# aiortc/aioquic

Hardware: AMD Instinct MI355X
Metric: GiB/s device-resident AEAD protect+unprotect, 1200B packets, 1/2/4/8 MI355X (higher is better)
Workload: dtype u8

## Files before the change

### aioquic_amd/csrc/qpp_device.h

```cpp
#pragma once

#include <hip/hip_runtime.h>
#include <stdint.h>

#include "../../include/quic_pp.h"
#include "qpp_gh5.h"
#include "qpp_te4.h"

namespace qpp {


extern __constant__ AesTables c_aes;


struct KeySlot {
    uint32_t suite;
    uint32_t key_phase;
    uint32_t nr;
    uint32_t rsv;
    uint32_t iv[4];
    uint32_t rk[60];
    uint32_t hrk[60];
    uint32_t rkr[60];
    uint32_t pad[4];
};
static_assert(sizeof(KeySlot) == 768, "KeySlot layout");

constexpr int kGhashPowers = 4;
constexpr int kGhashPowBytes = 32 * 16 * 16;

constexpr int kGh5Off = kGhashPowers * kGhashPowBytes;
constexpr int kGhPowCount = 192;
constexpr int kGhPowBytes = kGhPowCount * 16;
constexpr int kGhashTabBytes = kGh5Off + kGh5Bytes;
__device__ __host__ __forceinline__ size_t gh_powers_off(uint32_t cap, uint32_t slot)
{
    return (size_t)cap * kGhashTabBytes + (size_t)slot * kGhPowBytes;
}
// ... 180 lines not shown
        return (*(const uint32_t *)(te + addr<0>(s)) >> 8) & 0xffu;
    }
    __device__ __forceinline__ uint32_t f1(uint32_t s) const
    {
        return *(const uint32_t *)(te + addr<1>(s)) & 0xff00u;
    }
    __device__ __forceinline__ uint32_t f2(uint32_t s) const
    {
        return *(const uint32_t *)(te + 128 + addr<2>(s)) & 0xff0000u;
    }
    __device__ __forceinline__ uint32_t f3(uint32_t s) const
    {
        return *(const uint32_t *)(te + 128 + addr<3>(s)) & 0xff000000u;
    }
    __device__ __forceinline__ uint32_t fr0(uint32_t s) const { return *(const uint32_t *)(te + addr<0>(s)); }
    __device__ __forceinline__ uint32_t fr1(uint32_t s) const { return *(const uint32_t *)(te + addr<1>(s)); }
    __device__ __forceinline__ uint32_t fr2(uint32_t s) const { return *(const uint32_t *)(te + 128 + addr<2>(s)); }
    __device__ __forceinline__ uint32_t fr3(uint32_t s) const { return *(const uint32_t *)(te + 128 + addr<3>(s)); }
};

struct LdsTe4 {
    static constexpr bool kFourTables = true;
    const uint8_t *te;
    uint32_t lo;
    template <int R, bool HI>
    __device__ __forceinline__ uint32_t addr(uint32_t s) const
    {
        return __builtin_amdgcn_perm(s, lo, (HI ? 0x0c020000u : 0x0c0c0000u) | ((4u + R) << 8));
    }
    __device__ __forceinline__ uint32_t t0(uint32_t s) const { return *(const uint32_t *)(te + addr<0, false>(s)); }
    __device__ __forceinline__ uint32_t t1(uint32_t s) const { return *(const uint32_t *)(te + 128 + addr<1, false>(s)); }
    __device__ __forceinline__ uint32_t t2(uint32_t s) const { return *(const uint32_t *)(te + addr<2, true>(s)); }
    __device__ __forceinline__ uint32_t t3(uint32_t s) const { return *(const uint32_t *)(te + 128 + addr<3, true>(s)); }
    __device__ __forceinline__ uint32_t f0(uint32_t s) const { return (fr0(s) >> 8) & 0xffu; }
    __device__ __forceinline__ uint32_t f1(uint32_t s) const { return fr1(s) & 0xff00u; }
    __device__ __forceinline__ uint32_t f2(uint32_t s) const { return fr2(s) & 0xff0000u; }
    __device__ __forceinline__ uint32_t f3(uint32_t s) const { return fr3(s) & 0xff000000u; }
    __device__ __forceinline__ uint32_t fr0(uint32_t s) const { return *(const uint32_t *)(te + addr<0, false>(s)); }
    __device__ __forceinline__ uint32_t fr1(uint32_t s) const { return *(const uint32_t *)(te + addr<1, false>(s)); }
    __device__ __forceinline__ uint32_t fr2(uint32_t s) const { return *(const uint32_t *)(te + 128 + addr<2, false>(s)); }
    __device__ __forceinline__ uint32_t fr3(uint32_t s) const { return *(const uint32_t *)(te + 128 + addr<3, false>(s)); }
};

__device__ __forceinline__ uint32_t fin_col(uint32_t r0, uint32_t r1, uint32_t r2, uint32_t r3, uint32_t k)
{
    const uint32_t lo = __builtin_amdgcn_perm(r1, r0, 0x0c0c0501u);
    const uint32_t hi = __builtin_amdgcn_perm(r3, r2, 0x07020c0cu);
    return __builtin_amdgcn_bitop3_b32(lo, hi, k, 0x56);
}

struct ConstTe {
    __device__ __forceinline__ uint32_t t0(uint32_t s) const { return c_aes.te0[s & 255]; }
    __device__ __forceinline__ uint32_t t1(uint32_t s) const { return rotl(c_aes.te0[(s >> 8) & 255], 8); }
    __device__ __forceinline__ uint32_t t2(uint32_t s) const { return rotl(c_aes.te0[(s >> 16) & 255], 16); }
    __device__ __forceinline__ uint32_t t3(uint32_t s) const { return rotl(c_aes.te0[s >> 24], 24); }
    __device__ __forceinline__ uint32_t t2r(uint32_t s) const { return c_aes.te0[(s >> 16) & 255]; }
    __device__ __forceinline__ uint32_t t3r(uint32_t s) const { return rotl(c_aes.te0[s >> 24], 8); }
    __device__ __forceinline__ uint32_t f0(uint32_t s) const { return c_aes.sbox[s & 255]; }
    __device__ __forceinline__ uint32_t f1(uint32_t s) const { return (uint32_t)c_aes.sbox[(s >> 8) & 255] << 8; }
    __device__ __forceinline__ uint32_t f2(uint32_t s) const { return (uint32_t)c_aes.sbox[(s >> 16) & 255] << 16; }
    __device__ __forceinline__ uint32_t f3(uint32_t s) const { return (uint32_t)c_aes.sbox[s >> 24] << 24; }
};

template <int NR, int R0, bool KROT = false, class TE>
__device__ __forceinline__ u32x4 aes_rounds(u32x4 st, const uint32_t *rk, const TE &T)
{
// ... 60 lines not shown
    constexpr int kNext1 = 0x39, kNext2 = 0x4E, kNext3 = 0x93;
    uint32_t k[NR + 1];
#pragma unroll
    for (int r = 0; r <= NR; ++r) k[r] = rk[4 * r + sub];
    uint32_t s = (sub == 0 ? in.x : sub == 1 ? in.y : sub == 2 ? in.z : in.w) ^ k[0];
#pragma unroll
    for (int r = 1; r < NR; ++r) {
        const uint32_t s1 = quad_perm<kNext1>(s), s2 = quad_perm<kNext2>(s), s3 = quad_perm<kNext3>(s);
        s = xor3(xor3(T.t0(s), T.t1(s1), T.t2(s2)), T.t3(s3), k[r]);
    }
    const uint32_t s1 = quad_perm<kNext1>(s), s2 = quad_perm<kNext2>(s), s3 = quad_perm<kNext3>(s);
    s = (T.f0(s) | T.f1(s1) | T.f2(s2) | T.f3(s3)) ^ k[NR];
    return u32x4{quad_perm<0x00>(s), quad_perm<0x55>(s), quad_perm<0xAA>(s), quad_perm<0xFF>(s)};
}

struct CtrCache {
    uint32_t c0, d0, d1, d2, d3;
};

template <class TE>
__device__ __forceinline__ CtrCache ctr_cache(u32x4 nonce, const uint32_t *rk, const TE &T)
{
    const uint32_t s0 = nonce.x ^ rk[0], s1 = nonce.y ^ rk[1], s2 = nonce.z ^ rk[2], s3 = rk[3];
    const uint32_t c0 = xor3(T.t0(s0), T.t1(s1), T.t2(s2)) ^ rk[4];
    const uint32_t u1 = xor3(xor3(T.t0(s1), T.t1(s2), T.t2(s3)), T.t3(s0), rk[5]);
    const uint32_t u2 = xor3(xor3(T.t0(s2), T.t1(s3), T.t2(s0)), T.t3(s1), rk[6]);
    const uint32_t u3 = xor3(xor3(T.t0(s3), T.t1(s0), T.t2(s1)), T.t3(s2), rk[7]);
    return CtrCache{c0, xor3(T.t1(u1), T.t2(u2), T.t3(u3)) ^ rk[8],
                    xor3(T.t0(u1), T.t1(u2), T.t2(u3)) ^ rk[9],
                    xor3(T.t0(u2), T.t1(u3), T.t3(u1)) ^ rk[10],
                    xor3(T.t0(u3), T.t2(u1), T.t3(u2)) ^ rk[11]};
}

template <int NR, class TE>
__device__ __forceinline__ u32x4 aes_ctr(const CtrCache &c, uint32_t cb, const uint32_t *rk,
                                         const TE &T)
{
    const uint32_t u0 = c.c0 ^ T.t3(rk[3] ^ (cb << 24));
    const u32x4 v = {c.d0 ^ T.t0(u0), c.d1 ^ T.t3(u0), c.d2 ^ T.t2(u0), c.d3 ^ T.t1(u0)};
    return aes_rounds<NR, 3, true>(v, rk, T);
}

template <int NR, class TE>
__device__ __forceinline__ void aes_ctr2(const CtrCache &c, uint32_t cb0, uint32_t cb1,
                                         const uint32_t *rk, const TE &T, u32x4 &o0, u32x4 &o1)
{
    const uint32_t x0 = T.t3(rk[3] ^ (cb0 << 24)), x1 = T.t3(rk[3] ^ (cb1 << 24));
    __builtin_amdgcn_sched_barrier(0);
    const uint32_t u0 = c.c0 ^ x0, u1 = c.c0 ^ x1;
    const uint32_t v0 = T.t0(u0), v1 = T.t3(u0), v2 = T.t2(u0), v3 = T.t1(u0);
    const uint32_t w0 = T.t0(u1), w1 = T.t3(u1), w2 = T.t2(u1), w3 = T.t1(u1);
    __builtin_amdgcn_sched_barrier(0);
    uint32_t s[2][4] = {{c.d0 ^ v0, c.d1 ^ v1, c.d2 ^ v2, c.d3 ^ v3},
                        {c.d0 ^ w0, c.d1 ^ w1, c.d2 ^ w2, c.d3 ^ w3}};
#pragma unroll
    for (int r = 3; r < NR; ++r) {
        const uint32_t *k = rk + 4 * r;
        uint32_t e[2][16];
#pragma unroll
        for (int b = 0; b < 2; ++b) {
#pragma unroll
            for (int col = 0; col < 4; ++col) {
                e[b][4 * col + 0] = T.t0(s[b][col]);
                e[b][4 * col + 1] = T.t1(s[b][(col + 1) & 3]);
                if constexpr (TE::kFourTables) {
                    e[b][4 * col + 2] = T.t2(s[b][(col + 2) & 3]);
                    e[b][4 * col + 3] = T.t3(s[b][(col + 3) & 3]);
                } else {
                    e[b][4 * col + 2] = T.t2r(s[b][(col + 2) & 3]);
                    e[b][4 * col + 3] = T.t3r(s[b][(col + 3) & 3]);
                }
            }
        }
        __builtin_amdgcn_sched_barrier(0);
#pragma unroll
        for (int b = 0; b < 2; ++b) {
#pragma unroll
            for (int col = 0; col < 4; ++col) {
                if constexpr (TE::kFourTables)
                    s[b][col] = te_col4(e[b][4 * col], e[b][4 * col + 1], e[b][4 * col + 2], e[b][4 * col + 3], k[col]);
                else
                    s[b][col] = te_col2(e[b][4 * col], e[b][4 * col + 1], e[b][4 * col + 2], e[b][4 * col + 3], k[col]);
            }
        }
    }
    const uint32_t *k = rk + 4 * NR;
    uint32_t f[2][16];
#pragma unroll
    for (int b = 0; b < 2; ++b) {
#pragma unroll
        for (int col = 0; col < 4; ++col) {
            f[b][4 * col + 0] = T.fr0(s[b][col]);
            f[b][4 * col + 1] = T.fr1(s[b][(col + 1) & 3]);
            f[b][4 * col + 2] = T.fr2(s[b][(col + 2) & 3]);
            f[b][4 * col + 3] = T.fr3(s[b][(col + 3) & 3]);
        }
    }
    __builtin_amdgcn_sched_barrier(0);
    uint32_t o[2][4];
#pragma unroll
    for (int b = 0; b < 2; ++b) {
#pragma unroll
        for (int col = 0; col < 4; ++col)
            o[b][col] = fin_col(f[b][4 * col], f[b][4 * col + 1], f[b][4 * col + 2], f[b][4 * col + 3], k[col]);
    }
    o0 = u32x4{o[0][0], o[0][1], o[0][2], o[0][3]};
    o1 = u32x4{o[1][0], o[1][1], o[1][2], o[1][3]};
}


__device__ __forceinline__ u32x4 ghash_mul(u32x4 x, const uint8_t *lds, uint32_t tab)
{
    u32x4 acc = {0, 0, 0, 0};
    uint32_t xw[4] = {x.x, x.y, x.z, x.w};
#pragma unroll 1
    for (int d = 0; d < 4; ++d) {
        const uint32_t w = d == 0 ? xw[0] : d == 1 ? xw[1] : d == 2 ? xw[2] : xw[3];
        uint32_t hi = w & 0xF0F0F0F0u;
        uint32_t lo = (w << 4) & 0xF0F0F0F0u;
#pragma unroll
        for (int b = 0; b < 4; ++b) {
            const int wlo = 2 * (4 * d + b), whi = wlo + 1;
            const uint32_t sel = 0x0c0c0c00u | (uint32_t)b;
            uint32_t alo = __builtin_amdgcn_perm(0u, lo, sel);
            uint32_t ahi = __builtin_amdgcn_perm(0u, hi, sel);
            u32x4 e0 = *(const u32x4 *)(lds + tab + wlo * 256 + alo);
            u32x4 e1 = *(const u32x4 *)(lds + tab + whi * 256 + ahi);
            acc = xor3(acc, e0, e1);
        }
    }
    return acc;
}

template <int W0, int W1>
struct Gh5Grp {
    u32x2 lo[W1 - W0], hi[W1 - W0];
    __device__ __forceinline__ void issue(const uint32_t (&xw)[4], const uint8_t *base, uint32_t tsel)
    {
#pragma unroll
        for (int i = 0; i < W1 - W0; ++i) {
            const int w = W0 + i, sb = 5 * w, d = sb >> 5, off = sb & 31;
            uint32_t e;
            if (off <= 27) asm("v_bfe_u32 %0, %1, %2, 5" : "=v"(e) : "v"(xw[d]), "i"(off));
            else if (d < 3) e = __builtin_amdgcn_alignbit(xw[d + 1], xw[d], off) & 31u;
            else e = xw[3] >> off;
            const uint32_t a = (e << 3) | tsel;
            lo[i] = *(const u32x2 *)(base + w * 256 + a);
            hi[i] = *(const u32x2 *)(base + kGh5Hi + w * 256 + a);
        }
    }
    __device__ __forceinline__ void consume(u32x4 &acc) const
    {
        constexpr int n = W1 - W0;
#pragma unroll
        for (int i = 0; i + 1 < n; i += 2) {
            acc.x = xor3(acc.x, lo[i].x, lo[i + 1].x);
            acc.y = xor3(acc.y, lo[i].y, lo[i + 1].y);
            acc.z = xor3(acc.z, hi[i].x, hi[i + 1].x);
            acc.w = xor3(acc.w, hi[i].y, hi[i + 1].y);
        }
        if constexpr (n & 1) {
            acc.x ^= lo[n - 1].x;
            acc.y ^= lo[n - 1].y;
            acc.z ^= hi[n - 1].x;
            acc.w ^= hi[n - 1].y;
        }
    }
};

template <template <int, int> class Grp, class... In>
__device__ __forceinline__ u32x4 gh5_pipeline(const In &...in)
{
    u32x4 acc = {0, 0, 0, 0};
#define QPP_SB() __builtin_amdgcn_sched_barrier(0)
    {
        Grp<0, 5> a;
        Grp<5, 9> b;
        Grp<9, 14> c;
        Grp<14, 18> d;
        Grp<18, 22> e;
        Grp<22, kGh5Windows> f;
        a.issue(in...);
        b.issue(in...);
        QPP_SB();
        a.consume(acc);
        QPP_SB();
        c.issue(in...);
        QPP_SB();
        b.consume(acc);
        QPP_SB();
        d.issue(in...);
        QPP_SB();
        c.consume(acc);
        QPP_SB();
        e.issue(in...);
        QPP_SB();
        d.consume(acc);
        QPP_SB();
        f.issue(in...);
        QPP_SB();
        e.consume(acc);
        QPP_SB();
        f.consume(acc);
        QPP_SB();
    }
#undef QPP_SB
    return acc;
}
__device__ __forceinline__ u32x4 ghash_mul_lds5(u32x4 x, const uint8_t *base, uint32_t tsel)
{
    const uint32_t xw[4] = {x.x, x.y, x.z, x.w};
    return gh5_pipeline<Gh5Grp>(xw, base, tsel);
}

__device__ __forceinline__ u32x4 ghash_mul_h4(u32x4 x, const uint8_t *base, uint32_t tsel)
{
    return ghash_mul_lds5(x, base, tsel);
}

template <int W0, int W1>
struct Gh5GrpC : Gh5Grp<W0, W1> {
    template <int i = 0>
    __device__ __forceinline__ void issue(const Gh5In &in, const uint8_t *base)
    {
        if constexpr (i < W1 - W0) {
            constexpr int w = W0 + i;
            const uint32_t a = gh5_addr<w>(in);
            this->lo[i] = *(const u32x2 *)(base + w * 256 + a);
            this->hi[i] = *(const u32x2 *)(base + kGh5Hi + w * 256 + a);
            issue<i + 1>(in, base);
        }
    }
};
__device__ __forceinline__ u32x4 ghash_mul_lds5c(u32x4 x, const uint8_t *base)
{
    const Gh5In in(x.x, x.y, x.z, x.w);
    return gh5_pipeline<Gh5GrpC>(in, base);
}

__device__ __forceinline__ u32x4 ghash_mul_global(u32x4 x, const uint8_t *tab)
{
    u32x4 acc = {0, 0, 0, 0};
    uint32_t xw[4] = {x.x, x.y, x.z, x.w};
#pragma unroll 1
    for (int d = 0; d < 4; ++d) {
        const uint32_t w = d == 0 ? xw[0] : d == 1 ? xw[1] : d == 2 ? xw[2] : xw[3];
        uint32_t hi = w & 0xF0F0F0F0u;
        uint32_t lo = (w << 4) & 0xF0F0F0F0u;
#pragma unroll
        for (int b = 0; b < 4; ++b) {
            const int wlo = 2 * (4 * d + b), whi = wlo + 1;
            const uint32_t sel = 0x0c0c0c00u | (uint32_t)b;
            const uint32_t alo = __builtin_amdgcn_perm(0u, lo, sel);
            const uint32_t ahi = __builtin_amdgcn_perm(0u, hi, sel);
            u32x4 e0 = *(const u32x4 *)(tab + wlo * 256 + alo);
            u32x4 e1 = *(const u32x4 *)(tab + whi * 256 + ahi);
            acc = xor3(acc, e0, e1);
        }
    }
    return acc;
}

__device__ inline u32x4 gf128_mul_slow(u32x4 x, u32x4 y)
{
    uint64_t xh = (uint64_t)bswap(x.x) << 32 | bswap(x.y), xl = (uint64_t)bswap(x.z) << 32 | bswap(x.w);
    uint64_t vh = (uint64_t)bswap(y.x) << 32 | bswap(y.y), vl = (uint64_t)bswap(y.z) << 32 | bswap(y.w);
    uint64_t zh = 0, zl = 0;
    for (int i = 0; i < 128; ++i) {
        uint64_t bit = i < 64 ? (xh >> (63 - i)) & 1 : (xl >> (127 - i)) & 1;
        if (bit) { zh ^= vh; zl ^= vl; }
// ... 11 lines not shown
```

### aioquic_amd/csrc/qpp_engine.hip

```cpp
#include <hip/hip_runtime.h>

#include "qpp_chacha.h"
#include "qpp_gf128.h"
#include "qpp_device.h"
#include "qpp_hkdf.h"
#include "qpp_internal.h"
#include "qpp_phase.h"

namespace qpp {

__constant__ AesTables c_aes = kAesTables;

constexpr int kSetupWG = 256;
constexpr int kScratch = 112;
constexpr int kScrEj0 = 48, kScrPark = 64, kScrHdr = 96;
constexpr uint32_t kNoSlot = 0xffffffffu;
constexpr int kChachaWpe = 4;

constexpr int kChRegion = 64 * 16 + 16;
constexpr int kChStage = 4 * kChRegion;

constexpr int kPwOne = 0, kPw1 = 1, kPw8 = 6, kPw13 = 7, kPwEntries = 11;
constexpr int kChCarryAt = 7;

// ... 447 lines not shown
        }
        if (rb & 1) __builtin_amdgcn_raw_buffer_store_b8((unsigned char)t, r, o + (rb & 2), 0, 0);
    }
}

__device__ __forceinline__ void write_header_v(const Pkt &P, int sub, bool masked, int rlen, u32x4 h0,
                                               bool have_h0)
{
    const int n_a = (P.hlen + 15) >> 4;
    for (int q = sub; q < n_a; q += 4) {
        const int nb = min(16, P.hlen - 16 * q);
        u32x4 h = (q == 0 && have_h0) ? h0 : ld_win(P.src + 16 * q, nb, P.src, P.src + rlen);
        if (masked) h ^= hp_pattern(16 * q, P.mask, P.fbm, P.pn_off, P.pn_len);
        st_part(P.dst + 16 * q, h, nb);
    }
}

template <int NR, bool ENC, int BPL, int SUITE, bool PRIO, bool CLDS = false>
__device__ __forceinline__ u32x4 gcm_packet(const Pkt &P, const KeySlot *ks, const u32x4 h0,
                                            const uint32_t *rk, int sub, const GhashTabs &G,
                                            const uint8_t *te, const Bufs &B, uint32_t ioff, uint32_t ooff,
                                            u32x4 &got_tag)
{
    typedef std::conditional_t<CLDS, LdsTe4, LdsTe> Te;
    auto te_now = [&]() -> Te { return Te{te, (lane_fresh() & 31) * 4 | (CLDS ? 0x10000u : 0u)}; };
    const Te T = te_now();
    const int hlen = P.hlen, clen = P.clen;
    const int n_a = (hlen + 15) >> 4, n_c = (clen + 15) >> 4, za = n_a > 0 ? 1 : 0;
    const int n_g = za + n_c + 1, pad = gcm_pad<BPL>(n_g), S = (n_g + pad) / (4 * BPL);
    const int rlen = hlen + clen + (ENC ? 0 : QPP_TAG_LEN);
    const bool tiny = rlen < 16;
    const uint32_t t4 = CLDS ? 0u : G.t4();
    auto mul_h4 = [&](u32x4 x) -> u32x4 {
        if constexpr (CLDS) return ghash_mul_lds5c(x, G.lds);
        else return ghash_mul_h4(x, G.lds, t4);
    };
    const u32x4 tiny_in = tiny ? ld_part(P.src, rlen) : zero4();
    const int q = pad + za;
    const uint32_t cin = ioff + (uint32_t)hlen, cout = ooff + (uint32_t)hlen;
    auto ct_load = [&](int i) -> uint32_t {
        if (i < 0 || 16 * i >= clen) return kOob;
        return cin + (uint32_t)(ENC ? min(16 * i, clen - 16) : 16 * i);
    };
    u32x4 nxt0 = {0, 0, 0, 0}, nxt1 = {0, 0, 0, 0};
    if constexpr (BPL == 2) {
        nxt0 = __builtin_amdgcn_raw_buffer_load_b128(B.in, (int)ct_load(sub - q), 0, 0);
        nxt1 = __builtin_amdgcn_raw_buffer_load_b128(B.in, (int)ct_load(sub - q + 4), 0, 0);
    }

    auto mul_pow = [&](u32x4 x, uint32_t pw, auto two_c) -> u32x4 {
        if constexpr (CLDS) {
            if (G.close_resident()) {
                if constexpr (decltype(two_c)::value) {
                    const u32x4 m = ghash_mul(x, G.ctab, (uint32_t)kGhashPowBytes);
                    const bool two = (lane_fresh() & 2) == 0;
                    x = u32x4{two ? m.x : x.x, two ? m.y : x.y, two ? m.z : x.z, two ? m.w : x.w};
                    return ghash_mul(x, G.ctab, (lane_fresh() & 1) ? 0u : (uint32_t)kGhashPowBytes);
                } else {
                    return ghash_mul(x, G.ctab, pw * (uint32_t)kGhashPowBytes);
                }
            }
        }
        return ghash_mul_global(x, G.global(pw));
    };
    u32x4 z = {0, 0, 0, 0};
    for (int g = 0; g < n_a; ++g) {
        u32x4 a;
        if (tiny) {
            a = tiny_in;
        } else if (g == 0) {
            a = h0;
        } else {
            const int ld = min(16 * g, rlen - 16);
            a = shr_bytes(__builtin_amdgcn_raw_buffer_load_b128(B.in, (int)(ioff + ld), 0, 0),
                          16 * g - ld);
        }
        a = keep_bytes(a, min(16, hlen - 16 * g));
        if (!ENC && P.hp) a ^= hp_pattern(16 * g, P.mask, P.fbm, P.pn_off, P.pn_len);
        if (g > 0) z = mul_pow(z, 0u, std::false_type{});
        z ^= a;
    }
    if (!ENC || !P.hp) write_header_v(P, sub, !ENC && P.hp, rlen, tiny ? tiny_in : h0, true);
    const bool fast_hp = ENC && P.hp && gcm_fast_hp<BPL>(hlen, clen);
    u32x4 acc = (BPL == 1 && za && sub == pad) ? z : u32x4{0, 0, 0, 0};
    const CtrCache cc = ctr_cache(P.nonce, rk, T);
    const uint32_t lens_h = bswap((uint32_t)hlen * 8u);

    auto close = [&](u32x4 ksl) {
        const uint32_t lf = lane_fresh();
        acc = mul_pow(acc, 3u - (lf & 3), std::true_type{});
        if ((lf & 3) == 3) acc ^= ksl;
    };
    auto blk_out = [&](int i, u32x4 ksb, u32x4 raw) -> u32x4 {
        const bool is_ct = i >= 0 && 16 * i < clen;
        u32x4 x = {0, 0, 0, 0}, out = {0, 0, 0, 0};
        uint32_t soff = kOob;
        if (is_ct) {
            const int nb = clen - 16 * i;
            if (__builtin_expect(nb >= 16, 1)) {
                out = raw ^ ksb;
                x = ENC ? out : raw;
                soff = cout + 16u * (uint32_t)i;
            } else {
                const u32x4 cur = ENC ? shr_bytes(raw, 16 - nb) : raw;
                out = cur ^ ksb;
                x = keep_bytes(ENC ? out : cur, nb);
                buf_st_part(B.out, cout + 16u * (uint32_t)i, out, nb);
            }
        } else if (i >= 0 && 16 * i < clen + 16) {
            x = u32x4{0u, lens_h, 0u, bswap((uint32_t)clen * 8u)};
        }
        __builtin_amdgcn_raw_buffer_store_b128(out, B.out, (int)soff, 0, 0);
        return x;
    };
    auto step = [&](int i, bool last, auto first_c, u32x4 raw) {
        (void)first_c;
        const Te Tl = te_now();
        const bool is_ct = i >= 0 && 16 * i < clen;
        const u32x4 ksb = aes_ctr<NR>(cc, is_ct ? (uint32_t)(i + 2) : 1u, rk, Tl);
        acc ^= blk_out(i, ksb, raw);
        __builtin_amdgcn_sched_barrier(0);
        if (!last) acc = mul_h4(acc);
        else close(ksb);
    };
    auto step2 = [&](int i, bool last, u32x4 raw0, u32x4 raw1, auto first_c) {
        constexpr bool first = decltype(first_c)::value;
        const Te Tl = te_now();
        const uint32_t cb0 = (i >= 0 && 16 * i < clen) ? (uint32_t)(i + 2) : 1u;
        const uint32_t cb1 = (i + 4 >= 0 && 16 * (i + 4) < clen) ? (uint32_t)(i + 6) : 1u;
        u32x4 ks0, ks1;
        if (first && pad >= 4) {
            ks0 = zero4();
            ks1 = aes_ctr<NR>(cc, cb1, rk, Tl);
        } else {
            aes_ctr2<NR>(cc, cb0, cb1, rk, Tl, ks0, ks1);
        }
        u32x4 x0 = blk_out(i, ks0, raw0);
        u32x4 x1 = blk_out(i + 4, ks1, raw1);
        if constexpr (first) {
            if constexpr (ENC) {
                if (fast_hp) {
                    u32x4 c0 = (i == 0) ? x0 : (i + 4 == 0) ? x1 : zero4();
                    u32x4 c1 = (i == 1) ? x0 : (i + 4 == 1) ? x1 : zero4();
                    c0 = quad_xor_all(c0);
                    c1 = quad_xor_all(c1);
                    const int s = 4 - P.pn_len;
                    const u32x4 smp = {__builtin_amdgcn_alignbyte(c0.y, c0.x, s),
                                       __builtin_amdgcn_alignbyte(c0.z, c0.y, s),
                                       __builtin_amdgcn_alignbyte(c0.w, c0.z, s),
                                       __builtin_amdgcn_alignbyte(c1.x, c0.w, s)};
                    Pkt H = P;
                    H.mask = hp_mask_quad<SUITE>(ks, smp, Tl, sub);
                    write_header_v(H, sub, true, rlen, h0, true);
                }
            }
            if (i == -1) x0 ^= z;
            if (i + 4 == -1) x1 ^= z;
        }
        __builtin_amdgcn_sched_barrier(0);
        if (first && pad >= 4) acc = x1;
        else acc = mul_h4(acc ^ x0) ^ x1;
        if (!last) acc = mul_h4(acc);
        else close(ks1);
    };
    got_tag = u32x4{0, 0, 0, 0};
    if constexpr (BPL == 2) {
        if (tiny) {
            QPP_PROBE_AT(4);
            const u32x4 st = shl_bytes(tiny_in, 16 - rlen);
            step2(sub - q, true, st, st, std::true_type{});
        } else {
            int i = sub - q;
            auto one2 = [&](int k, auto first_c) {
                const u32x4 raw0 = nxt0, raw1 = nxt1;
                const uint32_t l0 = (!ENC && k == 1) ? cin + (uint32_t)clen : ct_load(i + 8);
                nxt0 = __builtin_amdgcn_raw_buffer_load_b128(B.in, (int)l0, 0, 0);
                nxt1 = __builtin_amdgcn_raw_buffer_load_b128(B.in, (int)ct_load(i + 12), 0, 0);
                step2(i, k == 1, raw0, raw1, first_c);
                i += 8;
            };
            constexpr int kInteriorK = 3;
            auto inner2 = [&]() {
                const u32x4 raw0 = nxt0, raw1 = nxt1;
                const uint32_t lo = cin + 16u * (uint32_t)i;
                nxt0 = __builtin_amdgcn_raw_buffer_load_b128(B.in, (int)(lo + 128u), 0, 0);
                nxt1 = __builtin_amdgcn_raw_buffer_load_b128(B.in, (int)(lo + 192u), 0, 0);
                const Te Tl = te_now();
                u32x4 ks0, ks1;
                aes_ctr2<NR>(cc, (uint32_t)(i + 2), (uint32_t)(i + 6), rk, Tl, ks0, ks1);
                const u32x4 out0 = raw0 ^ ks0, out1 = raw1 ^ ks1;
                const uint32_t so = cout + 16u * (uint32_t)i;
                __builtin_amdgcn_raw_buffer_store_b128(out0, B.out, (int)so, 0, 0);
                __builtin_amdgcn_raw_buffer_store_b128(out1, B.out, (int)(so + 64u), 0, 0);
                __builtin_amdgcn_sched_barrier(0);
                acc = mul_h4(mul_h4(acc ^ (ENC ? out0 : raw0)) ^ (ENC ? out1 : raw1));
                i += 8;
            };
            QPP_PROBE_AT(4);
            one2(S, std::true_type{});
#pragma unroll 1
            for (int k = S - 1; k > 0; --k) {
                if constexpr (PRIO) {
                    const int kr = __builtin_amdgcn_readfirstlane(k);
                    if (kr >= 7) __builtin_amdgcn_s_setprio(3);
                    else if (kr >= 4) __builtin_amdgcn_s_setprio(2);
                    else if (kr >= 2) __builtin_amdgcn_s_setprio(1);
                    else __builtin_amdgcn_s_setprio(0);
                }
                if (__builtin_amdgcn_ballot_w64(k < kInteriorK) == 0) inner2();
                else one2(k, std::false_type{});
            }
            if (!ENC) got_tag = nxt0;
        }
    } else if (tiny) {
        QPP_PROBE_AT(4);
        step(sub - q, true, std::true_type{}, shl_bytes(tiny_in, 16 - rlen));
    } else {
        int i = sub - q;
        auto in_of = [&](int k, int j) -> uint32_t {
            return (!ENC && k == 0) ? cin + (uint32_t)clen : ct_load(j);
        };
        u32x4 nxt = __builtin_amdgcn_raw_buffer_load_b128(B.in, (int)ct_load(i), 0, 0);
        QPP_PROBE_AT(4);
        auto one = [&](int k, auto first_c) {
            const u32x4 raw = nxt;
            nxt = __builtin_amdgcn_raw_buffer_load_b128(B.in, (int)in_of(k - 1, i + 4), 0, 0);
            step(i, k == 1, first_c, raw);
            i += 4;
        };
        one(S, std::true_type{});
#pragma unroll 1
        for (int k = S - 1; k > 0; --k) one(k, std::false_type{});
        if (!ENC) got_tag = nxt;
    }
    QPP_PROBE_AT(5);
    return quad_xor_all(acc);
}

template <bool ENC, int SUITE, int BPL>
__device__ __forceinline__ void gcm_finish(Pkt &P, const KeySlot *ks, int sub, const LdsTe &T, u32x4 tag,
                                           u32x4 got_tag)
{
    if (ENC) {
// ... 294 lines not shown
constexpr int kClosePowers = 2;
constexpr int kCloseTabBytes = kClosePowers * kGhashPowBytes;
static_assert(kClosePowers <= kGhashPowers && kCloseTabBytes % 1024 == 0 && kCloseTabBytes == 16 * 1024,
              "the close tables: 16 LDS-DMA pieces of 1 KiB, the head of the slot's 4-bit tables");

__device__ uint32_t g_qpp_watchdog;

__device__ uint32_t g_qpp_spin_tab = 1u << 22;
__device__ uint32_t g_qpp_spin_lone = 1u << 18;
__device__ uint32_t g_qpp_pair_delay = 0u;

template <int WG, bool CLDS = false, int NE = gcm_tab_entries<WG, CLDS>()>
struct __attribute__((aligned(16))) GcmSmem {
    static constexpr int kEntries = NE;
    static constexpr bool kClose = CLDS;
    uint8_t h4[NE][kGhLdsEntry];
    uint8_t ctab[CLDS ? kCloseTabBytes : 0];
    uint32_t cslot[CLDS ? 4 : 0];
    uint8_t te[CLDS ? 2 * kTeBytes : kTeBytes];
    uint32_t eslot[NE];
    uint32_t eref[NE];
    uint32_t eready[NE];
    uint32_t eused[NE];

    uint32_t lock, tick, next;
    uint32_t exited;
    uint32_t wslot[WG / 64];
    uint32_t went[WG / 64];
};

typedef GcmSmem<1024, true> GcmSmemClose;
static_assert(sizeof(GcmSmem<1024, true>) <= 163840, "the close-from-LDS form fits a workgroup's LDS");
static_assert(offsetof(GcmSmemClose, te) + 128 < 65536, "the image's base rides in the ds_read immediate");

template <class SM>
__device__ uint32_t tab_acquire(SM &sm, const uint8_t *gtab, uint32_t cur)
{
    const uint32_t spin = __builtin_nontemporal_load(&g_qpp_spin_tab);
    typedef const __attribute__((address_space(1))) void *gptr_t;
    typedef __attribute__((address_space(3))) void *lptr_t;
    uint32_t e = kNoSlot, load = 0;
#pragma unroll 1
    for (uint32_t it = 0; it < spin; ++it) {
        uint32_t got = kNoSlot, ld = 0;
        if (lane_fresh() == 0) {
            while (atomicCAS(&sm.lock, 0u, 1u) != 0u) __builtin_amdgcn_s_sleep(1);
            int hit = -1, vic = -1;
            uint32_t best = 0xffffffffu;
#pragma unroll
            for (int i = 0; i < SM::kEntries; ++i) {
                const uint32_t s = lds_ld(&sm.eslot[i]);
                const uint32_t r = lds_ld(&sm.eref[i]);
                const uint32_t u = lds_ld(&sm.eused[i]);
                if (s == cur) hit = i;
                else if (r == 0u && u < best) {
                    best = u;
                    vic = i;
                }
            }
            if (hit < 0 && vic >= 0) {
                hit = vic;
                ld = 1;
                lds_st(&sm.eslot[vic], cur);
                lds_st(&sm.eready[vic], 0u);
                if constexpr (SM::kClose) {
                    if (lds_ld(&sm.cslot[0]) == kNoSlot) {
// ... 1 lines not shown
                        ld = 3;
                    }
                }
            }
            if (hit >= 0) {
                got = (uint32_t)hit;
                atomicAdd(&sm.eref[hit], 1u);
                const uint32_t t = lds_ld(&sm.tick) + 1u;
                lds_st(&sm.tick, t);
                lds_st(&sm.eused[hit], t);
            }
            asm volatile("s_waitcnt lgkmcnt(0)" ::: "memory");
            atomicExch(&sm.lock, 0u);
        }
        got = __builtin_amdgcn_readfirstlane(got);
        if (got != kNoSlot) {
            e = got;
            load = __builtin_amdgcn_readfirstlane(ld);
            break;
        }
        __builtin_amdgcn_s_sleep(8);
    }
    if (e == kNoSlot) return e;
    if (load) {
        const uint8_t *src = gtab + (size_t)cur * kGhashTabBytes + kGh5Off;
        const uint32_t l = lane_fresh();
#pragma unroll
        for (int c = 0; c < kGhLdsEntry / 1024; ++c)
            __builtin_amdgcn_global_load_lds((gptr_t)(src + c * 1024 + l * 16), (lptr_t)(sm.h4[e] + c * 1024),
                                             16, 0, 0);
        if constexpr (SM::kClose) {
            if (load & 2u) {
                const uint8_t *src4 = gtab + (size_t)cur * kGhashTabBytes;
#pragma unroll 4
                for (int c = 0; c < kCloseTabBytes / 1024; ++c)
                    __builtin_amdgcn_global_load_lds((gptr_t)(src4 + c * 1024 + l * 16),
                                                     (lptr_t)(sm.ctab + c * 1024), 16, 0, 0);
            }
        }
        asm volatile("s_waitcnt vmcnt(0)" ::: "memory");
        if (lane_fresh() == 0) lds_st(&sm.eready[e], 1u);
    } else {
        bool ready = false;
#pragma unroll 1
        for (uint32_t it = 0; it < spin; ++it) {
            if (__builtin_amdgcn_readfirstlane(lds_ld(&sm.eready[e]))) {
                ready = true;
                break;
            }
            __builtin_amdgcn_s_sleep(2);
        }
        if (!ready) {
            if (lane_fresh() == 0) atomicSub(&sm.eref[e], 1u);
            return kNoSlot;
        }
    }
    return e;
}

template <class SM>
__device__ __forceinline__ void tab_release(SM &sm, uint32_t e)
{
    if (lane_fresh() == 0) atomicSub(&sm.eref[e], 1u);
}

constexpr uint32_t kPoolDiv = 12;

template <int SUITE, bool ENC, int WG, int BPL, bool CLDS = false>
__global__ __launch_bounds__(WG) __attribute__((amdgpu_waves_per_eu(4))) void k_gcm(const KeySlot *__restrict__ slots,
                                              const uint8_t *__restrict__ gtab, uint32_t cap,
// ... 1677 lines not shown
```

### aioquic_amd/build.py

```python

import hashlib
import os
import subprocess
import sys
import sysconfig

try:
    from . import _srchash
except ImportError:
    sys.path.insert(0, os.path.dirname(os.path.abspath(__file__)))
    import _srchash

PKG = os.path.dirname(os.path.abspath(__file__))
ROOT = os.path.dirname(PKG)
CSRC = os.path.join(PKG, "csrc")
INCLUDE = os.path.join(ROOT, "include")
OBJ = os.path.join(ROOT, "build", "obj")
LIB = os.path.join(PKG, "libquicpp.so")
EXT = os.path.join(PKG, "_crypto.abi3.so")
HIPCC = os.environ.get("HIPCC", "/opt/rocm/bin/hipcc")
ARCH = "gfx950"

COMMON_DEPS = ["qpp_batch.h", "qpp_device.h", "qpp_gh5.h", "qpp_internal.h", "qpp_te4.h"]
HIP_UNITS = {
    "qpp_engine.hip": ["qpp_chacha.h", "qpp_gf128.h", "qpp_hkdf.h", "qpp_phase.h", "qpp_route.h",
                       "qpp_sha_consts.h"],
    "qpp_plan.hip": [],
    "qpp_route.hip": ["qpp_accept.h", "qpp_route.h", "qpp_walk.h"],
    "qpp_session.hip": ["qpp_hostcopy.h"],
}


MARKER = b"qpp-source-hash:"
REPORT: dict = {}


def _inputs_hash(paths, flags=()):
    h = hashlib.sha256()
    for p in paths:
        h.update(os.path.basename(p).encode() + b"\0")
        with open(p, "rb") as f:
            h.update(f.read())
    h.update(repr(list(flags)).encode())
    return h.hexdigest()


def _stale(target, paths, flags=()):
    side = target + ".inputs"
    want = _inputs_hash(paths, flags)
    if not os.path.exists(target) or not os.path.exists(side):
        return True, want
    with open(side) as f:
        return f.read().strip() != want, want


def _record(target, want):
# ... 95 lines not shown
```

### aioquic_amd/csrc/qpp_te4.h

```cpp
#pragma once

#include <stdint.h>

#if defined(__HIPCC__)
#define QPP_TE4_HD __host__ __device__ __forceinline__
#else
#define QPP_TE4_HD inline
#endif

namespace qpp {

struct AesTables {
    uint8_t sbox[256];
    uint32_t te0[256];
};

constexpr uint8_t gf8_mul(uint8_t a, uint8_t b)
{
    uint8_t r = 0;
    for (int i = 0; i < 8; ++i) {
        if (b & 1) r ^= a;
        a = (uint8_t)((a << 1) ^ ((a & 0x80) ? 0x1b : 0));
        b >>= 1;
    }
// ... 25 lines not shown

QPP_TE4_HD uint32_t te_rotl(uint32_t x, int n)
{
#if defined(__HIP_DEVICE_COMPILE__)
    return __builtin_amdgcn_alignbit(x, x, (32 - n) & 31);
#else
    n &= 31;
    return n ? (x << n) | (x >> (32 - n)) : x;
#endif
}
QPP_TE4_HD uint32_t te_xor3(uint32_t a, uint32_t b, uint32_t c)
{
#if defined(__HIP_DEVICE_COMPILE__)
    return __builtin_amdgcn_bitop3_b32(a, b, c, 0x96);
#else
    return a ^ b ^ c;
#endif
}

QPP_TE4_HD uint32_t te_image_word(uint32_t te0, int half, int part)
{
    return te_rotl(te0, 16 * half + (part < 8 ? 0 : 8));
}

QPP_TE4_HD uint32_t te_col2(uint32_t e0, uint32_t e1, uint32_t e2r, uint32_t e3r, uint32_t kr)
{
    return te_xor3(e0, e1, te_rotl(te_xor3(e2r, e3r, kr), 16));
}
QPP_TE4_HD uint32_t te_col4(uint32_t e0, uint32_t e1, uint32_t e2, uint32_t e3, uint32_t k)
{
    return te_xor3(te_xor3(e0, e1, e2), e3, k);
}

}
```

Baseline: 498.7.

## Add explicit LDS waitcnts in AES/GHASH pipelines and restructure interior loop

```diff
diff --git a/aioquic_amd/csrc/qpp_device.h b/aioquic_amd/csrc/qpp_device.h
--- a/aioquic_amd/csrc/qpp_device.h
+++ b/aioquic_amd/csrc/qpp_device.h
@@ -385,16 +385,27 @@
     return aes_rounds<NR, 3, true>(v, rk, T);
 }
 
-template <int NR, class TE>
+constexpr int kWaitLdsOnly = 0xC07F;
+template <int N>
+__device__ __forceinline__ void lds_wait()
+{
+    static_assert(N >= 0 && N < 16, "lgkmcnt has four bits");
+    __builtin_amdgcn_s_waitcnt(kWaitLdsOnly | (N << 8));
+    __builtin_amdgcn_sched_barrier(0);
+}
+
+template <int NR, bool WAITS = false, class TE>
 __device__ __forceinline__ void aes_ctr2(const CtrCache &c, uint32_t cb0, uint32_t cb1,
                                          const uint32_t *rk, const TE &T, u32x4 &o0, u32x4 &o1)
 {
     const uint32_t x0 = T.t3(rk[3] ^ (cb0 << 24)), x1 = T.t3(rk[3] ^ (cb1 << 24));
     __builtin_amdgcn_sched_barrier(0);
+    if constexpr (WAITS) lds_wait<0>();
     const uint32_t u0 = c.c0 ^ x0, u1 = c.c0 ^ x1;
     const uint32_t v0 = T.t0(u0), v1 = T.t3(u0), v2 = T.t2(u0), v3 = T.t1(u0);
     const uint32_t w0 = T.t0(u1), w1 = T.t3(u1), w2 = T.t2(u1), w3 = T.t1(u1);
     __builtin_amdgcn_sched_barrier(0);
+    if constexpr (WAITS) lds_wait<0>();
     uint32_t s[2][4] = {{c.d0 ^ v0, c.d1 ^ v1, c.d2 ^ v2, c.d3 ^ v3},
                         {c.d0 ^ w0, c.d1 ^ w1, c.d2 ^ w2, c.d3 ^ w3}};
 #pragma unroll
@@ -419,6 +430,7 @@
         __builtin_amdgcn_sched_barrier(0);
 #pragma unroll
         for (int b = 0; b < 2; ++b) {
+            if constexpr (WAITS) b == 0 ? lds_wait<15>() : lds_wait<0>();
 #pragma unroll
             for (int col = 0; col < 4; ++col) {
                 if constexpr (TE::kFourTables)
@@ -444,6 +456,7 @@
     uint32_t o[2][4];
 #pragma unroll
     for (int b = 0; b < 2; ++b) {
+        if constexpr (WAITS) b == 0 ? lds_wait<15>() : lds_wait<0>();
 #pragma unroll
         for (int col = 0; col < 4; ++col)
             o[b][col] = fin_col(f[b][4 * col], f[b][4 * col + 1], f[b][4 * col + 2], f[b][4 * col + 3], k[col]);
@@ -478,6 +491,7 @@
 
 template <int W0, int W1>
 struct Gh5Grp {
+    static constexpr int kReads = 2 * (W1 - W0);
     u32x2 lo[W1 - W0], hi[W1 - W0];
     __device__ __forceinline__ void issue(const uint32_t (&xw)[4], const uint8_t *base, uint32_t tsel)
     {
@@ -512,11 +526,12 @@
     }
 };
 
-template <template <int, int> class Grp, class... In>
+template <template <int, int> class Grp, bool WAIT = false, class... In>
 __device__ __forceinline__ u32x4 gh5_pipeline(const In &...in)
 {
     u32x4 acc = {0, 0, 0, 0};
 #define QPP_SB() __builtin_amdgcn_sched_barrier(0)
+#define QPP_LW(next) do { if constexpr (WAIT) lds_wait<next>(); } while (0)
     {
         Grp<0, 5> a;
         Grp<5, 9> b;
@@ -527,39 +542,48 @@
         a.issue(in...);
         b.issue(in...);
         QPP_SB();
+        QPP_LW(decltype(b)::kReads);
         a.consume(acc);
         QPP_SB();
         c.issue(in...);
         QPP_SB();
+        QPP_LW(decltype(c)::kReads);
         b.consume(acc);
         QPP_SB();
         d.issue(in...);
         QPP_SB();
+        QPP_LW(decltype(d)::kReads);
         c.consume(acc);
         QPP_SB();
         e.issue(in...);
         QPP_SB();
+        QPP_LW(decltype(e)::kReads);
         d.consume(acc);
         QPP_SB();
         f.issue(in...);
         QPP_SB();
+        QPP_LW(decltype(f)::kReads);
         e.consume(acc);
         QPP_SB();
+        QPP_LW(0);
         f.consume(acc);
         QPP_SB();
     }
+#undef QPP_LW
 #undef QPP_SB
     return acc;
 }
+template <bool WAIT = false>
 __device__ __forceinline__ u32x4 ghash_mul_lds5(u32x4 x, const uint8_t *base, uint32_t tsel)
 {
     const uint32_t xw[4] = {x.x, x.y, x.z, x.w};
-    return gh5_pipeline<Gh5Grp>(xw, base, tsel);
-}
-
+    return gh5_pipeline<Gh5Grp, WAIT>(xw, base, tsel);
+}
+
+template <bool WAIT = false>
 __device__ __forceinline__ u32x4 ghash_mul_h4(u32x4 x, const uint8_t *base, uint32_t tsel)
 {
-    return ghash_mul_lds5(x, base, tsel);
+    return ghash_mul_lds5<WAIT>(x, base, tsel);
 }
 
 template <int W0, int W1>
@@ -576,10 +600,11 @@
         }
     }
 };
+template <bool WAIT = false>
 __device__ __forceinline__ u32x4 ghash_mul_lds5c(u32x4 x, const uint8_t *base)
 {
     const Gh5In in(x.x, x.y, x.z, x.w);
-    return gh5_pipeline<Gh5GrpC>(in, base);
+    return gh5_pipeline<Gh5GrpC, WAIT>(in, base);
 }
 
 __device__ __forceinline__ u32x4 ghash_mul_global(u32x4 x, const uint8_t *tab)
diff --git a/aioquic_amd/csrc/qpp_engine.hip b/aioquic_amd/csrc/qpp_engine.hip
--- a/aioquic_amd/csrc/qpp_engine.hip
+++ b/aioquic_amd/csrc/qpp_engine.hip
@@ -503,8 +503,8 @@
     const bool tiny = rlen < 16;
     const uint32_t t4 = CLDS ? 0u : G.t4();
     auto mul_h4 = [&](u32x4 x) -> u32x4 {
-        if constexpr (CLDS) return ghash_mul_lds5c(x, G.lds);
-        else return ghash_mul_h4(x, G.lds, t4);
+        if constexpr (CLDS) return ghash_mul_lds5c<BPL == 2>(x, G.lds);
+        else return ghash_mul_h4<BPL == 2>(x, G.lds, t4);
     };
     const u32x4 tiny_in = tiny ? ld_part(P.src, rlen) : zero4();
     const int q = pad + za;
@@ -594,7 +594,7 @@
         if (!last) acc = mul_h4(acc);
         else close(ksb);
     };
-    auto step2 = [&](int i, bool last, u32x4 raw0, u32x4 raw1, auto first_c) {
+    auto step2 = [&](int i, bool last, u32x4 raw0, u32x4 raw1, auto first_c, auto after_aes) {
         constexpr bool first = decltype(first_c)::value;
         const Te Tl = te_now();
         const uint32_t cb0 = (i >= 0 && 16 * i < clen) ? (uint32_t)(i + 2) : 1u;
@@ -604,8 +604,9 @@
             ks0 = zero4();
             ks1 = aes_ctr<NR>(cc, cb1, rk, Tl);
         } else {
-            aes_ctr2<NR>(cc, cb0, cb1, rk, Tl, ks0, ks1);
-        }
+            aes_ctr2<NR, true>(cc, cb0, cb1, rk, Tl, ks0, ks1);
+        }
+        after_aes();
         u32x4 x0 = blk_out(i, ks0, raw0);
         u32x4 x1 = blk_out(i + 4, ks1, raw1);
         if constexpr (first) {
@@ -639,15 +640,24 @@
         if (tiny) {
             QPP_PROBE_AT(4);
             const u32x4 st = shl_bytes(tiny_in, 16 - rlen);
-            step2(sub - q, true, st, st, std::true_type{});
+            step2(sub - q, true, st, st, std::true_type{}, [] {});
         } else {
             int i = sub - q;
             auto one2 = [&](int k, auto first_c) {
                 const u32x4 raw0 = nxt0, raw1 = nxt1;
-                const uint32_t l0 = (!ENC && k == 1) ? cin + (uint32_t)clen : ct_load(i + 8);
-                nxt0 = __builtin_amdgcn_raw_buffer_load_b128(B.in, (int)l0, 0, 0);
-                nxt1 = __builtin_amdgcn_raw_buffer_load_b128(B.in, (int)ct_load(i + 12), 0, 0);
-                step2(i, k == 1, raw0, raw1, first_c);
+                auto request = [&]() {
+                    const uint32_t l0 = (!ENC && k == 1) ? cin + (uint32_t)clen : ct_load(i + 8);
+                    nxt0 = __builtin_amdgcn_raw_buffer_load_b128(B.in, (int)l0, 0, 0);
+                    nxt1 = __builtin_amdgcn_raw_buffer_load_b128(B.in, (int)ct_load(i + 12), 0, 0);
+                };
+                constexpr bool late = decltype(first_c)::value && !CLDS;
+                if constexpr (!late) request();
+                step2(i, k == 1, raw0, raw1, first_c, [&]() {
+                    if constexpr (late) {
+                        __builtin_amdgcn_sched_barrier(0);
+                        request();
+                    }
+                });
                 i += 8;
             };
             constexpr int kInteriorK = 3;
@@ -658,7 +668,7 @@
                 nxt1 = __builtin_amdgcn_raw_buffer_load_b128(B.in, (int)(lo + 192u), 0, 0);
                 const Te Tl = te_now();
                 u32x4 ks0, ks1;
-                aes_ctr2<NR>(cc, (uint32_t)(i + 2), (uint32_t)(i + 6), rk, Tl, ks0, ks1);
+                aes_ctr2<NR, true>(cc, (uint32_t)(i + 2), (uint32_t)(i + 6), rk, Tl, ks0, ks1);
                 const u32x4 out0 = raw0 ^ ks0, out1 = raw1 ^ ks1;
                 const uint32_t so = cout + 16u * (uint32_t)i;
                 __builtin_amdgcn_raw_buffer_store_b128(out0, B.out, (int)so, 0, 0);
@@ -669,8 +679,7 @@
             };
             QPP_PROBE_AT(4);
             one2(S, std::true_type{});
-#pragma unroll 1
-            for (int k = S - 1; k > 0; --k) {
+            auto prio = [&](int k) {
                 if constexpr (PRIO) {
                     const int kr = __builtin_amdgcn_readfirstlane(k);
                     if (kr >= 7) __builtin_amdgcn_s_setprio(3);
@@ -678,8 +687,21 @@
                     else if (kr >= 2) __builtin_amdgcn_s_setprio(1);
                     else __builtin_amdgcn_s_setprio(0);
                 }
-                if (__builtin_amdgcn_ballot_w64(k < kInteriorK) == 0) inner2();
-                else one2(k, std::false_type{});
+            };
+            int k = S - 1;
+#pragma unroll 1
+            while (k > 0) {
+                if (__builtin_amdgcn_ballot_w64(k < kInteriorK) == 0) {
+#pragma unroll 1
+                    do {
+                        prio(k);
+                        inner2();
+                        --k;
+                    } while (__builtin_amdgcn_ballot_w64(k < kInteriorK) == 0);
+                }
+                prio(k);
+                one2(k, std::false_type{});
+                --k;
             }
             if (!ENC) got_tag = nxt0;
         }
```

Measured after the change: 502.4 (median of 6 runs). No clear change (+0.7%).

## Relayout close GHASH tables in LDS into 4-bit rows and quad-split CTR cache

Applied to the files above, without the earlier changes.

```diff
diff --git a/aioquic_amd/build.py b/aioquic_amd/build.py
--- a/aioquic_amd/build.py
+++ b/aioquic_amd/build.py
@@ -21,7 +21,7 @@
 HIPCC = os.environ.get("HIPCC", "/opt/rocm/bin/hipcc")
 ARCH = "gfx950"
 
-COMMON_DEPS = ["qpp_batch.h", "qpp_device.h", "qpp_gh5.h", "qpp_internal.h", "qpp_te4.h"]
+COMMON_DEPS = ["qpp_batch.h", "qpp_close4.h", "qpp_device.h", "qpp_gh5.h", "qpp_internal.h", "qpp_te4.h"]
 HIP_UNITS = {
     "qpp_engine.hip": ["qpp_chacha.h", "qpp_gf128.h", "qpp_hkdf.h", "qpp_phase.h", "qpp_route.h",
                        "qpp_sha_consts.h"],
diff --git a/aioquic_amd/csrc/qpp_close4.h b/aioquic_amd/csrc/qpp_close4.h
--- /dev/null
+++ b/aioquic_amd/csrc/qpp_close4.h
@@ -0,0 +1,64 @@
+#pragma once
+
+#include <stdint.h>
+
+#if defined(__HIPCC__)
+#define QPP_C4_HD __host__ __device__ __forceinline__
+#else
+#define QPP_C4_HD inline
+#endif
+
+namespace qpp {
+
+constexpr int kClose4Tables = 2;
+constexpr int kClose4Windows = 32;
+constexpr int kClose4RowBytes = 256;
+constexpr int kClose4TableBytes = 128;
+constexpr int kClose4Bytes = 2 * kClose4Windows * kClose4RowBytes;
+constexpr int kClose4SrcPowBytes = kClose4Windows * 16 * 16;
+
+constexpr int close4_table(int pw) { return 1 - pw; }
+constexpr int close4_row(int half, int w)
+{
+    return half == 0 ? w : kClose4Windows + (w & ~7) + ((w + 1) & 7);
+}
+constexpr int close4_off(int half, int table, int w, int e)
+{
+    return close4_row(half, w) * kClose4RowBytes + table * kClose4TableBytes + e * 8;
+}
+constexpr bool close4_mergeable(int dist)
+{
+    const int a = dist < 0 ? -dist : dist;
+    return (a % 8 == 0 && a / 8 <= 255) || (a % 512 == 0 && a / 512 <= 255);
+}
+constexpr bool close4_layout_ok()
+{
+    for (int w = 0; w < kClose4Windows; ++w) {
+        if (close4_mergeable(close4_off(1, 0, w, 0) - close4_off(0, 0, w, 0))) return false;
+        if (close4_row(1, w) < kClose4Windows || close4_row(1, w) >= 2 * kClose4Windows) return false;
+        if ((close4_row(1, w) - kClose4Windows) / 8 != w / 8) return false;
+    }
+    return true;
+}
+static_assert(close4_layout_ok(), "high halves: every row used once, no mergeable distance");
+
+QPP_C4_HD void close4_place(uint32_t idx, uint32_t &lo_off, uint32_t &hi_off)
+{
+    const int pw = (int)(idx >> 9), w = (int)(idx >> 4) & 31, e = (int)idx & 15;
+    lo_off = (uint32_t)close4_off(0, close4_table(pw), w, e);
+    hi_off = (uint32_t)close4_off(1, close4_table(pw), w, e);
+}
+
+QPP_C4_HD uint32_t close4_even(uint32_t x, uint32_t t4) { return ((x << 3) & 0x78787878u) | t4; }
+QPP_C4_HD uint32_t close4_odd(uint32_t x, uint32_t t4) { return ((x >> 1) & 0x78787878u) | t4; }
+QPP_C4_HD uint32_t close4_addr(uint32_t nib, int b, uint32_t d8 )
+{
+#if defined(__HIP_DEVICE_COMPILE__)
+    return __builtin_amdgcn_perm(d8, nib, 0x0c0c0400u | (uint32_t)b);
+#else
+    return ((nib >> (8 * b)) & 0xffu) | (d8 & 0xffu) << 8;
+#endif
+}
+constexpr int close4_imm(int half, int j) { return close4_row(half, j) * kClose4RowBytes; }
+
+}
diff --git a/aioquic_amd/csrc/qpp_device.h b/aioquic_amd/csrc/qpp_device.h
--- a/aioquic_amd/csrc/qpp_device.h
+++ b/aioquic_amd/csrc/qpp_device.h
@@ -4,6 +4,7 @@
 #include <stdint.h>
 
 #include "../../include/quic_pp.h"
+#include "qpp_close4.h"
 #include "qpp_gh5.h"
 #include "qpp_te4.h"
 
@@ -250,6 +251,10 @@
     __device__ __forceinline__ uint32_t t1(uint32_t s) const { return *(const uint32_t *)(te + 128 + addr<1, false>(s)); }
     __device__ __forceinline__ uint32_t t2(uint32_t s) const { return *(const uint32_t *)(te + addr<2, true>(s)); }
     __device__ __forceinline__ uint32_t t3(uint32_t s) const { return *(const uint32_t *)(te + 128 + addr<3, true>(s)); }
+    __device__ __forceinline__ uint32_t by_sel(uint32_t s, uint32_t sel, uint32_t lane_const) const
+    {
+        return *(const uint32_t *)(te + __builtin_amdgcn_perm(s, lane_const, sel));
+    }
     __device__ __forceinline__ uint32_t f0(uint32_t s) const { return (fr0(s) >> 8) & 0xffu; }
     __device__ __forceinline__ uint32_t f1(uint32_t s) const { return fr1(s) & 0xff00u; }
     __device__ __forceinline__ uint32_t f2(uint32_t s) const { return fr2(s) & 0xff0000u; }
@@ -376,6 +381,27 @@
                     xor3(T.t0(u3), T.t2(u1), T.t3(u2)) ^ rk[11]};
 }
 
+__device__ __forceinline__ CtrCache ctr_cache_quad(u32x4 nonce, const uint32_t *rk, const LdsTe4 &T, int sub)
+{
+    constexpr int kNext1 = 0x39, kNext2 = 0x4E, kNext3 = 0x93;
+    auto pick = [&](uint32_t a, uint32_t b, uint32_t c, uint32_t d) -> uint32_t {
+        return sub == 0 ? a : sub == 1 ? b : sub == 2 ? c : d;
+    };
+    const uint32_t s = pick(nonce.x ^ rk[0], nonce.y ^ rk[1], nonce.z ^ rk[2], rk[3]);
+    const uint32_t s1 = quad_perm<kNext1>(s), s2 = quad_perm<kNext2>(s), s3 = quad_perm<kNext3>(s);
+    const uint32_t e3 = T.t3(s3);
+    const uint32_t r1 = xor3(xor3(T.t0(s), T.t1(s1), T.t2(s2)), sub == 0 ? 0u : e3, pick(rk[4], rk[5], rk[6], rk[7]));
+    const uint32_t u1 = quad_perm<0x55>(r1), u2 = quad_perm<0xAA>(r1), u3 = quad_perm<0xFF>(r1);
+    const uint32_t lc = ctrq_lane_const(lane_fresh());
+    const uint32_t sel = pick(ctrq_sel(ctrq_table(0, 0)), ctrq_sel(ctrq_table(0, 1)), ctrq_sel(ctrq_table(0, 2)),
+                              ctrq_sel(ctrq_table(0, 3)));
+    const uint32_t e = xor3(T.by_sel(u1, quad_perm<kNext3>(sel), lc), T.by_sel(u2, quad_perm<kNext2>(sel), lc),
+                            T.by_sel(u3, quad_perm<kNext1>(sel), lc));
+    const uint32_t dj = e ^ pick(rk[8], rk[9], rk[10], rk[11]);
+    return CtrCache{quad_perm<0x00>(r1), quad_perm<0x00>(dj), quad_perm<0x55>(dj), quad_perm<0xAA>(dj),
+                    quad_perm<0xFF>(dj)};
+}
+
 template <int NR, class TE>
 __device__ __forceinline__ u32x4 aes_ctr(const CtrCache &c, uint32_t cb, const uint32_t *rk,
                                          const TE &T)
@@ -476,6 +502,40 @@
     return acc;
 }
 
+__device__ __forceinline__ u32x4 ghash_mul_close4(u32x4 x, const uint8_t *ctab, uint32_t t4)
+{
+    constexpr int kBatch = 4;
+    u32x4 acc = {0, 0, 0, 0};
+    uint32_t xw[4] = {x.x, x.y, x.z, x.w};
+#pragma unroll 1
+    for (int d = 0; d < 4; ++d) {
+        const uint32_t w = d == 0 ? xw[0] : d == 1 ? xw[1] : d == 2 ? xw[2] : xw[3];
+        const uint32_t ev = close4_even(w, t4), od = close4_odd(w, t4);
+        const uint32_t d8 = (uint32_t)d * 8u;
+#pragma unroll
+        for (int j0 = 0; j0 < 8; j0 += kBatch) {
+            u32x2 l[kBatch], h[kBatch];
+#pragma unroll
+            for (int i = 0; i < kBatch; ++i) {
+                const int j = j0 + i;
+                const uint32_t a = close4_addr((j & 1) ? od : ev, j >> 1, d8);
+                l[i] = *(const u32x2 *)(ctab + close4_imm(0, j) + a);
+                h[i] = *(const u32x2 *)(ctab + close4_imm(1, j) + a);
+            }
+            __builtin_amdgcn_sched_barrier(0);
+#pragma unroll
+            for (int i = 0; i < kBatch; i += 2) {
+                acc.x = xor3(acc.x, l[i].x, l[i + 1].x);
+                acc.y = xor3(acc.y, l[i].y, l[i + 1].y);
+                acc.z = xor3(acc.z, h[i].x, h[i + 1].x);
+                acc.w = xor3(acc.w, h[i].y, h[i + 1].y);
+            }
+            __builtin_amdgcn_sched_barrier(0);
+        }
+    }
+    return acc;
+}
+
 template <int W0, int W1>
 struct Gh5Grp {
     u32x2 lo[W1 - W0], hi[W1 - W0];
diff --git a/aioquic_amd/csrc/qpp_engine.hip b/aioquic_amd/csrc/qpp_engine.hip
--- a/aioquic_amd/csrc/qpp_engine.hip
+++ b/aioquic_amd/csrc/qpp_engine.hip
@@ -522,13 +522,15 @@
     auto mul_pow = [&](u32x4 x, uint32_t pw, auto two_c) -> u32x4 {
         if constexpr (CLDS) {
             if (G.close_resident()) {
+                constexpr uint32_t kH1 = 0x80808080u * (uint32_t)close4_table(0);
+                constexpr uint32_t kH2 = 0x80808080u * (uint32_t)close4_table(1);
                 if constexpr (decltype(two_c)::value) {
-                    const u32x4 m = ghash_mul(x, G.ctab, (uint32_t)kGhashPowBytes);
+                    const u32x4 m = ghash_mul_close4(x, G.ctab, kH2);
                     const bool two = (lane_fresh() & 2) == 0;
                     x = u32x4{two ? m.x : x.x, two ? m.y : x.y, two ? m.z : x.z, two ? m.w : x.w};
-                    return ghash_mul(x, G.ctab, (lane_fresh() & 1) ? 0u : (uint32_t)kGhashPowBytes);
+                    return ghash_mul_close4(x, G.ctab, (lane_fresh() & 1) ? kH1 : kH2);
                 } else {
-                    return ghash_mul(x, G.ctab, pw * (uint32_t)kGhashPowBytes);
+                    return ghash_mul_close4(x, G.ctab, pw ? kH2 : kH1);
                 }
             }
         }
@@ -554,7 +556,9 @@
     if (!ENC || !P.hp) write_header_v(P, sub, !ENC && P.hp, rlen, tiny ? tiny_in : h0, true);
     const bool fast_hp = ENC && P.hp && gcm_fast_hp<BPL>(hlen, clen);
     u32x4 acc = (BPL == 1 && za && sub == pad) ? z : u32x4{0, 0, 0, 0};
-    const CtrCache cc = ctr_cache(P.nonce, rk, T);
+    CtrCache cc;
+    if constexpr (CLDS) cc = ctr_cache_quad(P.nonce, rk, T, sub);
+    else cc = ctr_cache(P.nonce, rk, T);
     const uint32_t lens_h = bswap((uint32_t)hlen * 8u);
 
     auto close = [&](u32x4 ksl) {
@@ -1040,6 +1044,9 @@
 typedef GcmSmem<1024, true> GcmSmemClose;
 static_assert(sizeof(GcmSmem<1024, true>) <= 163840, "the close-from-LDS form fits a workgroup's LDS");
 static_assert(offsetof(GcmSmemClose, te) + 128 < 65536, "the image's base rides in the ds_read immediate");
+static_assert(kCloseTabBytes == kClose4Bytes && kClosePowers == kClose4Tables && kGhashPowBytes == kClose4SrcPowBytes,
+              "the close tables' copy: qpp_close4.h");
+static_assert(offsetof(GcmSmemClose, ctab) % kClose4RowBytes == 0, "a row of the copy spans the 64 banks once");
 
 template <class SM>
 __device__ uint32_t tab_acquire(SM &sm, const uint8_t *gtab, uint32_t cur)
@@ -1107,10 +1114,20 @@
         if constexpr (SM::kClose) {
             if (load & 2u) {
                 const uint8_t *src4 = gtab + (size_t)cur * kGhashTabBytes;
-#pragma unroll 4
-                for (int c = 0; c < kCloseTabBytes / 1024; ++c)
-                    __builtin_amdgcn_global_load_lds((gptr_t)(src4 + c * 1024 + l * 16),
-                                                     (lptr_t)(sm.ctab + c * 1024), 16, 0, 0);
+#pragma unroll 1
+                for (uint32_t c = 0; c < (uint32_t)kCloseTabBytes / 1024u; c += 4) {
+                    u32x4 v[4];
+#pragma unroll
+                    for (uint32_t i = 0; i < 4; ++i) v[i] = ld16(src4 + (c + i) * 1024u + l * 16u);
+#pragma unroll
+                    for (uint32_t i = 0; i < 4; ++i) {
+                        uint32_t lo_off, hi_off;
+                        close4_place((c + i) * 64u + l, lo_off, hi_off);
+                        *(u32x2 *)(sm.ctab + lo_off) = u32x2{v[i].x, v[i].y};
+                        *(u32x2 *)(sm.ctab + hi_off) = u32x2{v[i].z, v[i].w};
+                    }
+                }
+                asm volatile("s_waitcnt lgkmcnt(0)" ::: "memory");
             }
         }
         asm volatile("s_waitcnt vmcnt(0)" ::: "memory");
diff --git a/aioquic_amd/csrc/qpp_te4.h b/aioquic_amd/csrc/qpp_te4.h
--- a/aioquic_amd/csrc/qpp_te4.h
+++ b/aioquic_amd/csrc/qpp_te4.h
@@ -81,4 +81,14 @@
     return te_xor3(te_xor3(e0, e1, e2), e3, k);
 }
 
+constexpr int ctrq_table(int m, int j) { return (m - j) & 3; }
+constexpr uint32_t ctrq_sel(int r)
+{
+    return (r >= 2 ? 0x0c020000u : 0x0c0c0000u) | (uint32_t)(4 + r) << 8 | (uint32_t)(r & 1);
 }
+constexpr uint32_t ctrq_lane_const(uint32_t lane)
+{
+    return ((lane & 31u) * 4u) * 0x101u | 0x18000u;
+}
+
+}
```

After: 506.8 before, 510.9 after, median of 6. About the same (+0.8%).
